# openclimatefix/graph_weather

Hardware: NVIDIA H100
Metric: forward steps/sec (higher is better)
Workload: dtype f32 (fp16x2-split wgmma, fp32 accumulate)

## Files before the change

### graph_weather_b200/csrc/gw_tc3.cu

```cuda
#include <cuda_bf16.h>
#include <cuda_fp16.h>
#include <cuda_runtime.h>
#include <stdint.h>
#include <stdlib.h>

#include <algorithm>
#include <type_traits>

#include "gw_internal.h"
#include "gw_ops.h"
#include "gw_tc_ptx.cuh"

namespace gw {
namespace t3 {

#ifdef GW_ABLATE
#define ABL3(bit) ((ch.ablate & (bit)) != 0)
#else
#define ABL3(bit) false
#endif
#define GW_INLINE __attribute__((always_inline))
enum { ABL_FENCE = 1, ABL_LOADS = 2, ABL_CONVERT = 4, ABL_STORES = 8, ABL_LN = 16, ABL_WEIGHTS = 128 };

enum { F_ADD0 = 1, F_ADD1 = 2, F_RELU = 4, F_LN = 8, F_RES = 16, F_OUT = 32, F_FEEDS = 64, F_SEG = 128, F_NARROW = 256 };
// ... 42 lines not shown
    for (int k = 0; k < 2; ++k) p[k] = base + (size_t)(uint32_t)__ldg(s.idx + i0 + rl[k]) * ldb;
  } else {
#pragma unroll
    for (int k = 0; k < 2; ++k) p[k] = base + (size_t)(uint32_t)(i0 + rl[k]) * ldb;
  }
}
__device__ __forceinline__ void ld256(const char* p, float* o) {
  asm volatile("ld.global.nc.v4.f32 {%0, %1, %2, %3}, [%8];\n\t"
               "ld.global.nc.v4.f32 {%4, %5, %6, %7}, [%8+16];"
               : "=f"(o[0]), "=f"(o[1]), "=f"(o[2]), "=f"(o[3]), "=f"(o[4]), "=f"(o[5]), "=f"(o[6]), "=f"(o[7])
               : "l"(p));
}
__device__ __forceinline__ void st256(char* p, float a, float b, float c, float d, float e, float f, float g, float h) {
  asm volatile("st.global.v4.f32 [%0], {%1, %2, %3, %4};\n\t"
               "st.global.v4.f32 [%0+16], {%5, %6, %7, %8};" ::"l"(p), "f"(a), "f"(b), "f"(c), "f"(d), "f"(e), "f"(f), "f"(g), "f"(h)
               : "memory");
}
__device__ __forceinline__ void load8(const float* rowp, int col, int width, float* o) {
  const float* p = rowp + col;
  if (col + 8 <= width && (reinterpret_cast<uintptr_t>(p) & 31) == 0) {
    ld256(reinterpret_cast<const char*>(p), o);
  } else if (col + 8 <= width && (reinterpret_cast<uintptr_t>(p) & 15) == 0) {
    const float4 a = __ldg(reinterpret_cast<const float4*>(p)), b = __ldg(reinterpret_cast<const float4*>(p + 4));
    o[0] = a.x, o[1] = a.y, o[2] = a.z, o[3] = a.w, o[4] = b.x, o[5] = b.y, o[6] = b.z, o[7] = b.w;
  } else {
#pragma unroll
    for (int t = 0; t < 8; ++t) o[t] = (col + t < width) ? __ldg(p + t) : 0.f;
  }
}
__device__ __forceinline__ const float* src_row(const RowSrc& s, int b, int i0, int r) {
  const int i = src_gathered(s.kind) ? __ldg(s.idx + i0 + r) : i0 + r;
  return reinterpret_cast<const float*>(src_sample_base(s, b)) + (size_t)(uint32_t)i * (size_t)s.ld;
}
__host__ __device__ constexpr int FR(int m, int t) { return 4 * (t >> 1) + 2 * m + (t & 1); }
__host__ __device__ constexpr int PX(int i) { return 8 * ((i >> 1) & 1) + 2 * (i >> 2) + (i & 1); }
__device__ __forceinline__ float4 lds128(uint32_t addr) {
  float4 v;
  asm volatile("ld.shared.v4.f32 {%0, %1, %2, %3}, [%4];" : "=f"(v.x), "=f"(v.y), "=f"(v.z), "=f"(v.w) : "r"(addr));
  return v;
}
__device__ __forceinline__ float col8(const float4& lo, const float4& hi, int i) {
  const int c = 2 * (i >> 2) + (i & 1);
  const float4& b = (c & 4) ? hi : lo;
  return (c & 2) ? ((c & 1) ? b.w : b.z) : ((c & 1) ? b.y : b.x);
}
__device__ __forceinline__ void sts32(uint32_t addr, uint32_t v) { asm volatile("st.shared.b32 [%0], %1;" ::"r"(addr), "r"(v) : "memory"); }
template <bool SPLIT, bool ROWORDER>
__device__ __forceinline__ void store_operand_x4(uint32_t sa, const float (&v)[16], float& amax) {
#pragma unroll
  for (int m = 0; m < 2; ++m)
#pragma unroll
    for (int g = 0; g < 4; ++g) {
      const int i = ROWORDER ? 8 * m + 2 * g : 4 * g + 2 * m;
      const float a0 = v[i], a1 = v[i + 1];
      amax = fmaxf(amax, fmaxf(fabsf(a0), fabsf(a1)));
      const uint32_t addr = (sa ^ (uint32_t)(g << 4)) + 1024u * m;
      if (SPLIT) {
        const __half2 hh = __floats2half2_rn(a0, a1);
        const float2 hf = __half22float2(hh);
        const __half2 ll = __floats2half2_rn(a0 - hf.x, a1 - hf.y);
        sts32(addr, *reinterpret_cast<const uint32_t*>(&hh));
        sts32(addr + A_HALF_BYTES, *reinterpret_cast<const uint32_t*>(&ll));
      } else {
        const __nv_bfloat162 bb = __floats2bfloat162_rn(a0, a1);
        sts32(addr, *reinterpret_cast<const uint32_t*>(&bb));
      }
    }
}

__device__ __forceinline__ float fit_scale(float m) {
  if (!(m > 0.f) || !(m < 3.0e38f)) return 1.f;
  int e = (int)((__float_as_uint(m) >> 23) & 0xffu) - 127;
  e = e < -110 ? -110 : e;
  return __uint_as_float((uint32_t)(127 + 14 - e) << 23);
}
__device__ __forceinline__ float ldbound(const float* p) { return p ? __ldg(p) : 0.f; }
__device__ __forceinline__ float srcbound(const RowSrc& s) {
  if (!s.bound) return 0.f;
  const float m = __ldg(s.bound) * s.bound_mul;
  return s.bound_mul_i ? m * (float)max(__ldg(s.bound_mul_i), 1) : m;
}

template <bool SPLIT, int N>
__device__ __forceinline__ void mma_chunks(float (&d)[128], uint32_t a_rows, uint32_t b_base, uint32_t bar_full_b, uint32_t bar_empty_b,
                                           uint32_t& bi, int kc0, int kc1) {
  for (int kc = kc0; kc < kc1; ++kc) {
    const uint32_t a_hi = a_rows + (uint32_t)(kc % A_SLOTS) * A_SLOT_BYTES, a_lo = a_hi + A_HALF_BYTES;
#pragma unroll
    for (int part = 0; part < (SPLIT ? 2 : 1); ++part) {
      const uint32_t stage = bi % B_STAGES, nb = bi / B_STAGES;
      mbar_wait_or_trap(bar_full_b + 8 * stage, nb & 1);
      const uint32_t b = b_base + stage * B_STAGE_BYTES;
      wgmma_fence();
      if (part == 0) {
#pragma unroll
        for (int ks = 0; ks < 4; ++ks) Wgmma<N, !SPLIT>::mma(d, gmma_desc(a_hi + 32 * ks), gmma_desc(b + 32 * ks), (kc | ks) != 0);
        if (SPLIT) {
#pragma unroll
          for (int ks = 0; ks < 4; ++ks) Wgmma<N, !SPLIT>::mma(d, gmma_desc(a_lo + 32 * ks), gmma_desc(b + 32 * ks), 1);
        }
      } else {
#pragma unroll
        for (int ks = 0; ks < 4; ++ks) Wgmma<N, !SPLIT>::mma(d, gmma_desc(a_hi + 32 * ks), gmma_desc(b + 32 * ks), 1);
      }
      wgmma_commit();
      wgmma_wait<0>();
      mbar_arrive(bar_empty_b + 8 * stage);
      ++bi;
    }
  }
  fence_operand(d);
}

template <bool SPLIT, int MODE>
__global__ void __launch_bounds__(NUM_THREADS, 1) gw_chain_tc3_kernel(const __grid_constant__ TcChain ch) {
  extern __shared__ __align__(1024) uint8_t smem[];
  const uint32_t sbase = smem_u32(smem);
  const int warp = threadIdx.x >> 5, lane = threadIdx.x & 31;
  const int rows = ch.rows_per_sample, batch = ch.batch;
  const int tiles_per_sample = (rows + TILE_M - 1) / TILE_M;
  const int num_tiles = tiles_per_sample * batch;
  constexpr int parts = SPLIT ? 2 : 1;

  const uint32_t bar_full_b = sbase + OFF_BAR;
  const uint32_t bar_empty_b = bar_full_b + 8 * B_STAGES;

  if (threadIdx.x == 0) {
    if (sbase & 1023u) {
      if (ch.status) atomicOr(ch.status, 4);
      __trap();
    }
    for (int i = 0; i < B_STAGES; ++i) mbar_init(bar_full_b + 8 * i, 1), mbar_init(bar_empty_b + 8 * i, NUM_WORKERS);
    fence_barrier_init();
  }
  {
    float* par = reinterpret_cast<float*>(smem + OFF_PAR);
    float* lnp = reinterpret_cast<float*>(smem + OFF_LNP);
    int ln_slot = 0;
    for (int l = 0; l < ch.n_layers; ++l) {
      const TcLayer& L = ch.layer[l];
      for (int c = threadIdx.x; c < 256; c += NUM_THREADS) par[l * 256 + c] = (L.bias && c < L.n_valid) ? __ldg(L.bias + c) : 0.f;
      if (L.ln_g) {
        for (int c = threadIdx.x; c < 256; c += NUM_THREADS) {
          lnp[(ln_slot * 2 + 0) * 256 + c] = (c < L.n_valid) ? __ldg(L.ln_g + c) : 0.f;
          lnp[(ln_slot * 2 + 1) * 256 + c] = (c < L.n_valid) ? __ldg(L.ln_b + c) : 0.f;
        }
        ++ln_slot;
      }
    }
  }
  if (threadIdx.x == 32) {
    float* scl = reinterpret_cast<float*>(smem + OFF_SCL);
    float m = fmaxf(srcbound(ch.a0[0]), srcbound(ch.a0[1]));
    if (ch.a0[0].kind == SRC_GATHER_BCAST_RELU) m += ldbound(ch.a0[0].bound2);
    float sc = fit_scale(m);
    bool bad = !(m < 3.0e38f);
    scl[2 * PAR_LAYERS] = sc;
    for (int l = 0; l < ch.n_layers; ++l) {
      const TcLayer& L = ch.layer[l];
      const float wa = ldbound(L.wamax);
      const float winv = L.wamax ? 1.f / tc_weight_scale(wa, ch.split ? 2 : 1) : L.wscale_inv, gain = L.wamax ? (float)L.K * wa : L.gain;
      scl[2 * l] = winv / sc;
      const float pre = fmaf(m, gain, L.off) + srcbound(L.add[0]) + srcbound(L.add[1]);
      float mo = L.ln_g ? L.ln_bound : pre;
      mo += srcbound(L.residual);
      bad = bad || !(mo < 3.0e38f) || !(pre < 3.0e38f);
      if (blockIdx.x == 0) {
        if (L.out_bound) {
          const bool again = l > 0 && ch.layer[l - 1].out_bound == L.out_bound;
          *L.out_bound = again ? fmaxf(*L.out_bound, mo) : mo;
        }
        if (L.seg_bound) *L.seg_bound = mo * L.seg_maxdeg + ldbound(L.seg_add_bound);
      }
      float so = 1.f;
      if (L.feeds_next) {
        m = mo;
        sc = so = fit_scale(m);
      }
      scl[2 * l + 1] = so;
    }
    if (bad && ch.status) atomicOr(ch.status, 8);
  }
  __syncthreads();
  if (warp >= CONSUMER_WARPS) {
    asm volatile("setmaxnreg.dec.sync.aligned.u32 %0;" ::"n"(AUX_REGS));
    if (warp == WARP_PRODUCER && lane == 0) {
      uint32_t bi = 0;
      Tracer tr;
      tr.init(ch.trace, 0, true);
      for (int tile = blockIdx.x; tile < num_tiles; tile += gridDim.x) {
        for (int l = 0; l < ch.n_layers; ++l) {
          const TcLayer& L = ch.layer[l];
          const uint32_t panel = (uint32_t)L.N * 128u;
// ... 86 lines not shown
    row_ptrs2(ch.a0[0], bs, i0, r2, fcofs, pa);
    if constexpr (GBR) {
#pragma unroll
      for (int m = 0; m < 2; ++m) pb[m] = reinterpret_cast<const char*>(ch.a0[0].base2 + (size_t)(uint32_t)(i0 + r2[m]) * (size_t)ch.a0[0].ld2 + fcofs);
    } else if constexpr (NC1 > 0) {
      row_ptrs2(ch.a0[1], bs, i0, r2, fcofs, pb);
    }
    float buf[DEPTH][16] = {};
    float bufb[GBR ? DEPTH : 1][16] = {};
    auto fetch = [&](auto uu) GW_INLINE {
      constexpr int u = decltype(uu)::value, k = (u - U0) % DEPTH;
      if (ABL3(ABL_LOADS)) return;
      if constexpr (GBR) {
        ld256(pa[0] + 128 * u, buf[k]), ld256(pa[1] + 128 * u, buf[k] + 8);
        ld256(pb[0] + 128 * u, bufb[k]), ld256(pb[1] + 128 * u, bufb[k] + 8);
      } else if constexpr (u < 2 * NC0) {
        ld256(pa[0] + 128 * u, buf[k]), ld256(pa[1] + 128 * u, buf[k] + 8);
      } else {
        ld256(pb[0] + 128 * (u - 2 * NC0), buf[k]), ld256(pb[1] + 128 * (u - 2 * NC0), buf[k] + 8);
      }
    };
    static_for<U0, (U1 < U0 + DEPTH ? U1 : U0 + DEPTH)>([&](auto uu) GW_INLINE { fetch(uu); });
    static_for<U0, U1>([&](auto uu) GW_INLINE {
      constexpr int u = decltype(uu)::value, k = (u - U0) % DEPTH;
      float(&cur)[16] = buf[k];
      if constexpr (GBR) {
#pragma unroll
        for (int i = 0; i < 16; ++i) cur[i] = fmaxf(cur[i] + bufb[k][i], 0.f);
      }
      if (a0scale != 1.f) {
#pragma unroll
        for (int i = 0; i < 16; ++i) cur[i] *= a0scale;
      }
      if (!ABL3(ABL_CONVERT)) store_operand_x4<SPLIT, true>(op_addr(u), cur, amax);
      if constexpr (u + DEPTH < U1) fetch(ic<u + DEPTH>{});
    });
    publish();
  };

  auto bias_in_place = [&](float (&acc)[128], int l, int nu, float wsi) GW_INLINE {
    const uint32_t bias_a = sbase + OFF_PAR + l * 1024 + 4 * fcofs;
    static_for<0, 8>([&](auto uu) GW_INLINE {
      constexpr int u = decltype(uu)::value;
      if (u < nu) {
        const float4 bl = lds128(bias_a + 128 * u), bh = lds128(bias_a + 128 * u + 16);
#pragma unroll
        for (int i = 0; i < 16; ++i) acc[16 * u + i] = fmaf(acc[16 * u + i], wsi, col8(bl, bh, i));
      }
    });
  };
  auto ln_stats = [&](float (&acc)[128], int nu, int nval, float (&rs)[2], float (&sh)[2]) GW_INLINE {
    float s[2] = {0.f, 0.f};
    static_for<0, 8>([&](auto uu) GW_INLINE {
      constexpr int u = decltype(uu)::value;
      if (u < nu) {
#pragma unroll
        for (int i = 0; i < 16; ++i) s[(i >> 1) & 1] += acc[16 * u + i];
      }
    });
#pragma unroll
    for (int m = 0; m < 2; ++m) s[m] += __shfl_xor_sync(0xffffffffu, s[m], 1), s[m] += __shfl_xor_sync(0xffffffffu, s[m], 2);
    const float inv = 1.0f / (float)nval;
    const float mean[2] = {s[0] * inv, s[1] * inv};
    float v2[2] = {0.f, 0.f};
    static_for<0, 8>([&](auto uu) GW_INLINE {
      constexpr int u = decltype(uu)::value;
      if (u < nu) {
#pragma unroll
        for (int i = 0; i < 16; ++i) {
          const int m = (i >> 1) & 1;
          const float d = (32 * u + fcofs + 2 * (i >> 2) + (i & 1) < nval) ? acc[16 * u + i] - mean[m] : 0.f;
          v2[m] = fmaf(d, d, v2[m]);
        }
      }
    });
#pragma unroll
    for (int m = 0; m < 2; ++m) {
      v2[m] += __shfl_xor_sync(0xffffffffu, v2[m], 1), v2[m] += __shfl_xor_sync(0xffffffffu, v2[m], 2);
      const float rstd = 1.0f / sqrtf(v2[m] * inv + 1e-5f);
      rs[m] = rstd, sh[m] = -mean[m] * rstd;
    }
  };

  auto layer_fast = [&](float (&acc)[128], auto FLc, auto NPc, int l, int tile, int ln_slot) GW_INLINE {
    constexpr int F = decltype(FLc)::value, NP = decltype(NPc)::value, NU = 2 * NP;
    constexpr bool has_add0 = (F & F_ADD0) != 0, has_add1 = (F & F_ADD1) != 0, has_res = (F & F_RES) != 0, has_out = (F & F_OUT) != 0;
    constexpr bool relu = (F & F_RELU) != 0, has_ln = (F & F_LN) != 0, feeds = (F & F_FEEDS) != 0, has_seg = (F & F_SEG) != 0;
    constexpr bool has0 = has_add0 || has_res;
    const TcLayer& L = ch.layer[l];
    const int bs = tile % batch, i0 = (tile / batch) * TILE_M;
    const int nvalid = min(TILE_M, rows - i0);
    const float wsi = scl[2 * l], osc = scl[2 * l + 1];
    const uint32_t g_a = sbase + OFF_LNP + 4 * fcofs + (ln_slot * 2) * 1024, b_a = g_a + 1024;
    const RowSrc& src0 = has_add0 ? L.add[0] : L.residual;
    const char* p0[2] = {nullptr, nullptr};
    const char* p1[2] = {nullptr, nullptr};
    float pf0[16] = {}, pf1[16] = {};
    const bool ld_on = !ABL3(ABL_LOADS);
    auto ld2 = [&](const char* const(&p)[2], int off, float(&o)[16]) GW_INLINE { ld256(p[0] + off, o), ld256(p[1] + off, o + 8); };
    {
      const int r2[2] = {min(fr0, nvalid - 1), min(fr0 + 1, nvalid - 1)};
      if constexpr (has0) row_ptrs2(src0, bs, i0, r2, fcofs, p0);
      if constexpr (has_add1) row_ptrs2(L.add[1], bs, i0, r2, fcofs, p1);
    }
    if constexpr (has0) {
      if (ld_on) ld2(p0, 0, pf0);
    }
    if constexpr (has_add1) {
      if (ld_on) ld2(p1, 0, pf1);
    }
    int d0 = 0, d1 = 0, dprev_g = 0;
    if constexpr (has_seg) {
      const int32_t* sd = L.seg_dst + i0;
      d0 = (fr0 < nvalid) ? __ldg(sd + fr0) : -1;
      d1 = (fr0 + 1 < nvalid) ? __ldg(sd + fr0 + 1) : -2;
      dprev_g = (lr == 0 && i0 + frow > 0 && frow < nvalid) ? __ldg(sd + frow - 1) : -8;
    }
    bias_in_place(acc, l, NU, wsi);
    float rs[2] = {1.f, 1.f}, sh[2] = {0.f, 0.f};
    if constexpr (has_ln) {
      if (!ABL3(ABL_LN)) ln_stats(acc, NU, 64 * NP, rs, sh);
    }
    char* po = nullptr;
    const size_t ostr = 4 * (size_t)L.ldo;
    const bool st0 = fr0 < nvalid, st1 = fr0 + 1 < nvalid;
    if constexpr (has_out) po = reinterpret_cast<char*>(L.out + ((size_t)bs * rows + i0 + fr0) * (size_t)L.ldo + fcofs);
    bool bb = false, tail_st = false, head_st = false, one_st = false, one_any = false, deep = false;
    float mbf = 1.f, c1f = 0.f, e2f = 0.f, e4f = 0.f, kf = 0.f, k1f = 0.f;
    char* tail_p = nullptr;
    char* carry_p = nullptr;
    const char* add_p = nullptr;
    if constexpr (has_seg) {
      int dprev = __shfl_up_sync(0xffffffffu, d1, 4);
      if (lr == 0) dprev = dprev_g;
      const bool ba = d0 != dprev;
      bb = d1 != d0;
      mbf = bb ? 0.f : 1.f;
      const uint32_t nba = __shfl_down_sync(0xffffffffu, (uint32_t)ba, 4);
      const bool c1 = lr < 7 && !nba;
      const bool k = c1 && !bb;
      const uint32_t k1 = __shfl_down_sync(0xffffffffu, (uint32_t)k, 4), k2 = __shfl_down_sync(0xffffffffu, (uint32_t)k, 8);
      const uint32_t k3 = __shfl_down_sync(0xffffffffu, (uint32_t)k, 12);
      const bool e2 = c1 && k1;
      const bool e4 = e2 && k2 && k3;
      c1f = c1 ? 1.f : 0.f, e2f = e2 ? 1.f : 0.f, e4f = e4 ? 1.f : 0.f, kf = k ? 1.f : 0.f, k1f = (k && k1) ? 1.f : 0.f;
      deep = L.seg_maxdeg > 7;
      carry_p = reinterpret_cast<char*>(L.seg_carry + ((((size_t)bs * tiles_per_sample + (size_t)(i0 / TILE_M)) * 8 + (size_t)(frow >> 4)) * 256 + fcofs));
      if (ba || bb) {
        tail_st = d1 >= 0;
        tail_p = reinterpret_cast<char*>(L.seg_out + ((size_t)bs * L.seg_rows + (size_t)(uint32_t)max(d1, 0)) * (size_t)L.seg_ld + fcofs);
      } else if (lr == 0) {
        tail_st = d1 >= 0;
        tail_p = carry_p;
      }
      head_st = lr == 0 && !ba && bb && d0 >= 0;
      one_st = ba && bb && d0 >= 0;
      one_any = __any_sync(0xffffffffu, one_st);
      if (L.seg_add && (ba || bb) && d1 >= 0)
        add_p = reinterpret_cast<const char*>(L.seg_add + (size_t)(uint32_t)d1 * (size_t)L.seg_ld + fcofs);
    }
    static_for<0, NU>([&](auto uu) GW_INLINE {
      constexpr int u = decltype(uu)::value;
      float v[16];
#pragma unroll
      for (int i = 0; i < 16; ++i) v[i] = acc[16 * u + i];
      [[maybe_unused]] float sadd[8] = {0.f, 0.f, 0.f, 0.f, 0.f, 0.f, 0.f, 0.f};
      if constexpr (has_seg) {
        if (add_p) ld256(add_p + 128 * u, sadd);
      }
      if constexpr (has_add0) {
        if (ld_on) {
#pragma unroll
          for (int i = 0; i < 16; ++i) v[i] += pf0[PX(i)];
        }
      }
      if constexpr (has_add1) {
        if (ld_on) {
#pragma unroll
          for (int i = 0; i < 16; ++i) v[i] += pf1[PX(i)];
        }
      }
      if constexpr (relu) {
#pragma unroll
        for (int i = 0; i < 16; ++i) v[i] = fmaxf(v[i], 0.f);
      }
      if constexpr (has_ln) {
        const float4 gl = lds128(g_a + 128 * u), gh = lds128(g_a + 128 * u + 16);
        const float4 el = lds128(b_a + 128 * u), eh = lds128(b_a + 128 * u + 16);
#pragma unroll
        for (int i = 0; i < 16; ++i) {
          const int m = (i >> 1) & 1;
          v[i] = fmaf(fmaf(v[i], rs[m], sh[m]), col8(gl, gh, i), col8(el, eh, i));
        }
      }
      if constexpr (has_res) {
        if (ld_on) {
#pragma unroll
          for (int i = 0; i < 16; ++i) v[i] += pf0[PX(i)];
        }
      }
      if constexpr (u + 1 < NU) {
        if constexpr (has0) {
          if (ld_on) ld2(p0, 128 * (u + 1), pf0);
        }
        if constexpr (has_add1) {
          if (ld_on) ld2(p1, 128 * (u + 1), pf1);
        }
      }
      if constexpr (has_out) {
        if (!ABL3(ABL_STORES)) {
          if (st0) st256(po + 128 * u, v[FR(0, 0)], v[FR(0, 1)], v[FR(0, 2)], v[FR(0, 3)], v[FR(0, 4)], v[FR(0, 5)], v[FR(0, 6)], v[FR(0, 7)]);
          if (st1) st256(po + ostr + 128 * u, v[FR(1, 0)], v[FR(1, 1)], v[FR(1, 2)], v[FR(1, 3)], v[FR(1, 4)], v[FR(1, 5)], v[FR(1, 6)], v[FR(1, 7)]);
        }
      }
      if constexpr (has_seg) {
        float T[8], H[8];
#pragma unroll
        for (int t = 0; t < 8; ++t) {
          const float xa = v[FR(0, t)], xb = v[FR(1, t)];
          T[t] = fmaf(mbf, xa, xb);
          H[t] = bb ? xa : T[t];
        }
        const bool sts_on = !ABL3(ABL_STORES);
        if (head_st && sts_on) st256(carry_p + 128 * u, H[0], H[1], H[2], H[3], H[4], H[5], H[6], H[7]);
        if (one_any) {
          if (one_st && sts_on) {
            char* dp = reinterpret_cast<char*>(L.seg_out + ((size_t)bs * L.seg_rows + (size_t)(uint32_t)d0) * (size_t)L.seg_ld + fcofs);
            float a1[8] = {0.f, 0.f, 0.f, 0.f, 0.f, 0.f, 0.f, 0.f};
            if (L.seg_add) ld256(reinterpret_cast<const char*>(L.seg_add + (size_t)(uint32_t)d0 * (size_t)L.seg_ld + fcofs) + 128 * u, a1);
            st256(dp + 128 * u, H[0] + a1[0], H[1] + a1[1], H[2] + a1[2], H[3] + a1[3], H[4] + a1[4], H[5] + a1[5], H[6] + a1[6], H[7] + a1[7]);
          }
        }
#pragma unroll
        for (int t = 0; t < 8; ++t) {
          const float h1 = __shfl_down_sync(0xffffffffu, H[t], 4);
          T[t] = fmaf(c1f, h1, T[t]);
          H[t] = fmaf(kf, h1, H[t]);
        }
#pragma unroll
        for (int t = 0; t < 8; ++t) T[t] = fmaf(e2f, __shfl_down_sync(0xffffffffu, H[t], 8), T[t]);
        if (deep) {
#pragma unroll
          for (int t = 0; t < 8; ++t) {
            const float g2 = fmaf(k1f, __shfl_down_sync(0xffffffffu, H[t], 8), H[t]);
            T[t] = fmaf(e4f, __shfl_down_sync(0xffffffffu, g2, 16), T[t]);
          }
        }
        if (tail_st && sts_on)
          st256(tail_p + 128 * u, T[0] + sadd[0], T[1] + sadd[1], T[2] + sadd[2], T[3] + sadd[3], T[4] + sadd[4], T[5] + sadd[5], T[6] + sadd[6],
                T[7] + sadd[7]);
      }
      if constexpr (feeds) {
        if (osc != 1.f) {
#pragma unroll
          for (int i = 0; i < 16; ++i) v[i] *= osc;
        }
        if (!ABL3(ABL_CONVERT)) store_operand_x4<SPLIT, false>(op_addr(u), v, amax);
      }
      tr.ev(700 + 10 * l + u);
    });
    if constexpr (feeds) publish();
  };

  auto layer_out_narrow = [&](float (&acc)[128], int l, int tile) GW_INLINE {
    const TcLayer& L = ch.layer[l];
    const int bs = tile % batch, i0 = (tile / batch) * TILE_M;
    const int nvalid = min(TILE_M, rows - i0);
    const int nu = L.N >> 5, nval = L.n_valid;
    const bool has_res = L.residual.kind != SRC_NONE;
    const float* rp[2] = {nullptr, nullptr};
    if (has_res) {
      const float* base = reinterpret_cast<const float*>(src_sample_base(L.residual, bs));
#pragma unroll
      for (int m = 0; m < 2; ++m) rp[m] = base + (size_t)(uint32_t)(i0 + min(fr0 + m, nvalid - 1)) * (size_t)L.residual.ld;
    }
    float* op[2];
#pragma unroll
    for (int m = 0; m < 2; ++m) op[m] = L.out + ((size_t)bs * rows + i0 + fr0 + m) * (size_t)L.ldo;
    const bool st[2] = {fr0 < nvalid, fr0 + 1 < nvalid};
    bias_in_place(acc, l, nu, scl[2 * l]);
    static_for<0, 8>([&](auto uu) GW_INLINE {
      constexpr int u = decltype(uu)::value;
      const int c0 = 32 * u + fcofs;
      if (u < nu && 32 * u < nval) {
        float2 r[2][4] = {};
        if (has_res && !ABL3(ABL_LOADS)) {
#pragma unroll
          for (int m = 0; m < 2; ++m)
#pragma unroll
// ... 77 lines not shown
          *reinterpret_cast<float*>(reinterpret_cast<char*>(p) + (reinterpret_cast<const char*>(ch.out_peer[j]) - reinterpret_cast<const char*>(L.out))) = a;
      }
    };
    static_for<0, 8>([&](auto uu) GW_INLINE {
      constexpr int u = decltype(uu)::value;
      if (u < nu) {
        const int col = 32 * u + fcofs;
        const bool ld_ok = !ABL3(ABL_LOADS);
        float v[16];
#pragma unroll
        for (int i = 0; i < 16; ++i) v[i] = acc[16 * u + i];
        float t[16];
        if (has_add0 && ld_ok) {
          load8(q0[0], col, src0.width, t), load8(q0[1], col, src0.width, t + 8);
#pragma unroll
          for (int i = 0; i < 16; ++i) v[i] += t[PX(i)];
        }
        if (has_add1 && ld_ok) {
          load8(q1[0], col, L.add[1].width, t), load8(q1[1], col, L.add[1].width, t + 8);
#pragma unroll
          for (int i = 0; i < 16; ++i) v[i] += t[PX(i)];
        }
        if (relu) {
#pragma unroll
          for (int i = 0; i < 16; ++i) v[i] = fmaxf(v[i], 0.f);
        }
        if (has_pre && !ABL3(ABL_STORES)) store8(L.save_pre, v, col);
        if (has_ln) {
          const float4 gl = lds128(g_a + 128 * u), gh = lds128(g_a + 128 * u + 16);
          const float4 el = lds128(b_a + 128 * u), eh = lds128(b_a + 128 * u + 16);
#pragma unroll
          for (int i = 0; i < 16; ++i) {
            const int m = (i >> 1) & 1;
            v[i] = fmaf(fmaf(v[i], rs[m], sh[m]), col8(gl, gh, i), col8(el, eh, i));
          }
        }
        if (!has_add0 && has_res && ld_ok) {
          load8(q0[0], col, src0.width, t), load8(q0[1], col, src0.width, t + 8);
#pragma unroll
          for (int i = 0; i < 16; ++i) v[i] += t[PX(i)];
        }
        if (has_mask) {
          load8(src_row(L.mask, bs, i0, r2[0]), col, L.mask.width, t), load8(src_row(L.mask, bs, i0, r2[1]), col, L.mask.width, t + 8);
#pragma unroll
          for (int i = 0; i < 16; ++i) v[i] = t[PX(i)] > 0.f ? v[i] : 0.f;
        }
        if (nval < L.N) {
#pragma unroll
          for (int i = 0; i < 16; ++i)
            if (col + 2 * (i >> 2) + (i & 1) >= nval) v[i] = 0.f;
        }
        if (has_out && !ABL3(ABL_STORES)) {
#pragma unroll
          for (int m = 0; m < 2; ++m) {
            if (fr0 + m < nvalid) {
              float* orow = L.out + ((size_t)bs * rows + i0 + fr0 + m) * (size_t)L.ldo + col;
              if (col + 8 <= L.out_cols && (reinterpret_cast<uintptr_t>(orow) & 15) == 0) {
                put4(orow, v[FR(m, 0)], v[FR(m, 1)], v[FR(m, 2)], v[FR(m, 3)]);
                put4(orow + 4, v[FR(m, 4)], v[FR(m, 5)], v[FR(m, 6)], v[FR(m, 7)]);
              } else {
#pragma unroll
                for (int k = 0; k < 8; ++k)
                  if (col + k < L.out_cols) put1(orow + k, v[FR(m, k)]);
              }
            }
          }
        }
        if (feeds) {
          if (osc != 1.f) {
#pragma unroll
            for (int i = 0; i < 16; ++i) v[i] *= osc;
          }
          if (!ABL3(ABL_CONVERT)) store_operand_x4<SPLIT, false>(op_addr(u), v, amax);
        }
      }
    });
    if (feeds) publish();
  };

  auto run_layer = [&](auto Nc, int l, int tile, int ln_slot) GW_INLINE {
    constexpr int N = decltype(Nc)::value;
    const TcLayer& L = ch.layer[l];
    float acc[128];
    auto mma = [&](int kc0, int kc1) GW_INLINE {
      tr.ev(100 + kc0);
      mma_chunks<SPLIT, N>(acc, a_rows, sbase + OFF_B, bar_full_b, bar_empty_b, bi, kc0, kc1);
      wg_sync();
      tr.ev(110 + kc0);
    };
    if (l == 0) {
      const int nk0 = ch.K0 >> 6;
      for (int w = 0; 4 * w < nk0; ++w) {
        tr.ev(480 + w);
        if constexpr (MODE >= 1) {
          if (ch.a0[1].kind != SRC_NONE) {
            if (w == 0) stage0_fast(ic<4>{}, ic<4>{}, ic<0>{}, ic<0>{}, tile);
            else stage0_fast(ic<4>{}, ic<4>{}, ic<0>{}, ic<1>{}, tile);
          } else if (ch.a0[0].kind == SRC_GATHER_BCAST_RELU) {
            stage0_fast(ic<4>{}, ic<0>{}, ic<1>{}, ic<0>{}, tile);
          } else if (ch.K0 == 256) {
            stage0_fast(ic<4>{}, ic<0>{}, ic<0>{}, ic<0>{}, tile);
          } else {
            stage0_fast(ic<2>{}, ic<0>{}, ic<0>{}, ic<0>{}, tile);
          }
        } else {
          stage0(tile, w);
        }
        mma(4 * w, min(nk0, 4 * w + 4));
      }
    } else {
      mma(0, L.K >> 6);
    }
    if constexpr (MODE >= 1) {
      if constexpr (MODE == 2) {
        if (L.kind & F_NARROW) {
          layer_out_narrow(acc, l, tile);
          return;
        }
      }
#define GW_LF(M, NP_) case (M): layer_fast(acc, ic<(M)>{}, ic<(NP_)>{}, l, tile, ln_slot); break
      if constexpr (N == 256) {
        switch (L.kind) {
          GW_LF(F_ADD0 | F_ADD1 | F_RELU | F_FEEDS, 4);
          GW_LF(F_ADD0 | F_RELU | F_FEEDS, 4);
          GW_LF(F_RELU | F_FEEDS, 4);
          GW_LF(F_LN | F_RES | F_OUT, 4);
          GW_LF(F_LN | F_RES | F_OUT | F_SEG, 4);
          GW_LF(F_LN | F_RES | F_SEG, 4);
          GW_LF(F_LN | F_SEG, 4);
          GW_LF(F_LN | F_RES | F_OUT | F_FEEDS, 4);
          GW_LF(F_LN | F_FEEDS, 4);
          GW_LF(F_OUT, 4);
          GW_LF(F_RELU | F_OUT, 4);
          default: break;
        }
      } else {
        switch (L.kind) {
          GW_LF(F_RELU | F_FEEDS, 2);
          GW_LF(F_RELU | F_OUT, 2);
          default: break;
        }
      }
#undef GW_LF
    } else {
      layer_gen(acc, l, tile, ln_slot, l + 1 == ch.n_layers);
    }
  };

  const int n_layers = ch.n_layers;
  for (int tile = blockIdx.x; tile < num_tiles; tile += gridDim.x) {
    int ln_slot = 0;
    for (int l = 0; l < n_layers; ++l) {
      const int N = ch.layer[l].N;
      if constexpr (MODE >= 1) {
        if (N == 256) run_layer(ic<256>{}, l, tile, ln_slot);
        else run_layer(ic<128>{}, l, tile, ln_slot);
      } else {
        if (N == 256) run_layer(ic<256>{}, l, tile, ln_slot);
        else if (N == 192) run_layer(ic<192>{}, l, tile, ln_slot);
        else if (N == 128) run_layer(ic<128>{}, l, tile, ln_slot);
        else run_layer(ic<64>{}, l, tile, ln_slot);
      }
      if (ch.layer[l].ln_g) ++ln_slot;
      tr.ev(900 + l);
    }
  }
  if (SPLIT && ch.status && amax > 60000.f) atomicOr(ch.status, 1);
}

}

static bool aligned32(const void* p) { return (reinterpret_cast<uintptr_t>(p) & 31) == 0; }
static bool simple_kind(int k) { return k == SRC_STREAM || k == SRC_BCAST || k == SRC_GATHER || k == SRC_BGATHER; }
static bool fits32(const RowSrc& s) {
  const bool g = s.kind == SRC_GATHER || s.kind == SRC_BGATHER || s.kind == SRC_GATHER_BCAST_RELU;
  const long long span = g ? (long long)s.src_rows : 128;
  return span * (long long)s.ld * 4 + 4096 < (1ll << 32);
}
static bool src_fast(const RowSrc& s, int need) {
  return simple_kind(s.kind) && s.width >= need && aligned32(s.base + s.col0) && !(s.ld & 7) && fits32(s);
}

static void tc3_mark_lean(TcChain& ch) {
  using namespace t3;
  ch.fast = 0;
  {
    bool ok = true;
    int wsum = 0;
    for (int a = 0; a < 2; ++a) {
      const RowSrc& s = ch.a0[a];
      if (s.kind == SRC_NONE) continue;
      const bool gbr = s.kind == SRC_GATHER_BCAST_RELU;
      ok = ok && (simple_kind(s.kind) || gbr) && aligned32(s.base + s.col0) && !(s.ld & 7);
      if (gbr) ok = ok && aligned32(s.base2) && !(s.ld2 & 7);
      wsum += s.width;
    }
    const bool two = ch.a0[1].kind != SRC_NONE;
    ok = ok && ch.a0[0].kind != SRC_NONE && wsum == ch.K0;
    ok = ok && (two ? (ch.a0[0].width == 256 && ch.a0[1].width == 256) : (ch.K0 == 256 || ch.K0 == 128));
    if (ch.a0[0].kind == SRC_GATHER_BCAST_RELU) ok = ok && !two && ch.K0 == 256;
    if (ok) ch.fast |= (int32_t)0x80000000u;
  }
  static const int kinds4[] = {F_ADD0 | F_ADD1 | F_RELU | F_FEEDS, F_ADD0 | F_RELU | F_FEEDS, F_RELU | F_FEEDS, F_LN | F_RES | F_OUT,
                               F_LN | F_RES | F_OUT | F_SEG, F_LN | F_RES | F_SEG, F_LN | F_SEG, F_LN | F_RES | F_OUT | F_FEEDS, F_LN | F_FEEDS, F_OUT,
                               F_RELU | F_OUT};
  static const int kinds2[] = {F_RELU | F_FEEDS, F_RELU | F_OUT};
  for (int l = 0; l < ch.n_layers; ++l) {
    const TcLayer& L = ch.layer[l];
    if (L.save_pre || L.mask.kind != SRC_NONE) {
      ch.layer[l].kind = -1;
      continue;
    }
    const bool narrow = l + 1 == ch.n_layers && L.n_valid < L.N32 && !(L.n_valid & 1) && (L.N32 == 128 || L.N32 == 256) && L.out && !L.relu &&
                        !L.ln_g && !L.feeds_next && !L.seg_dst && L.add[0].kind == SRC_NONE && L.add[1].kind == SRC_NONE &&
                        !(reinterpret_cast<uintptr_t>(L.out) & 7) && !(L.ldo & 1) && L.out_cols >= L.n_valid &&
                        (L.residual.kind == SRC_NONE ||
                         ((L.residual.kind == SRC_STREAM || L.residual.kind == SRC_BCAST) && L.residual.width >= L.n_valid && !(L.residual.ld & 1) &&
                          !(reinterpret_cast<uintptr_t>(L.residual.base + L.residual.col0) & 7) && fits32(L.residual)));
    if (narrow) {
      ch.layer[l].kind = F_NARROW | F_OUT | (L.residual.kind != SRC_NONE ? F_RES : 0);
      ch.fast |= 1 << l;
      continue;
    }
    bool ok = (L.N == 256 || L.N == 128) && L.n_valid == L.N;
    for (int a = 0; a < 2; ++a)
      if (L.add[a].kind != SRC_NONE) ok = ok && src_fast(L.add[a], L.N);
    if (L.residual.kind != SRC_NONE) ok = ok && src_fast(L.residual, L.N);
    if (L.out) ok = ok && aligned32(L.out) && !(L.ldo & 7) && L.out_cols >= L.N;
    if (L.seg_dst) ok = ok && L.seg_out && L.seg_carry && aligned32(L.seg_out) && aligned32(L.seg_carry) && !(L.seg_ld & 7) && L.ln_g && L.N == 256;
    if (L.seg_add) ok = ok && L.seg_dst && aligned32(L.seg_add);
    const int f = (L.add[0].kind != SRC_NONE ? F_ADD0 : 0) | (L.add[1].kind != SRC_NONE ? F_ADD1 : 0) | (L.relu ? F_RELU : 0) |
                  (L.ln_g ? F_LN : 0) | (L.residual.kind != SRC_NONE ? F_RES : 0) | (L.out ? F_OUT : 0) | (L.feeds_next ? F_FEEDS : 0) |
                  (L.seg_dst ? F_SEG : 0);
    bool listed = false;
    if (L.N == 256) {
      for (int k : kinds4) listed = listed || k == f;
    } else {
      for (int k : kinds2) listed = listed || k == f;
    }
    ch.layer[l].kind = listed ? f : -1;
    if (ok && listed) ch.fast |= 1 << l;
  }
}
bool tc3_chain_is_lean(const TcChain& ch_in) {
  TcChain ch = ch_in;
  tc3_mark_lean(ch);
  if (getenv("GW_TC3_NOFAST")) return false;
  const int32_t all = (int32_t)(0x80000000u | ((1u << ch.n_layers) - 1u));
  return ch.fast == all && ch.out_mode == 0;
}
cudaError_t tc_column_block(const TcChain& ch, int n0, int nb, TcChain* out) {
  const TcLayer& L = ch.layer[0];
  if (ch.n_layers != 1 || n0 < 0 || nb <= 0 || nb > TC_COL_BLOCK || n0 + nb > L.n_valid) return cudaErrorInvalidValue;
  if (L.ln_g && (n0 != 0 || nb != L.n_valid)) return cudaErrorInvalidValue;
  if (L.feeds_next || L.seg_dst || ch.out_mode != 0) return cudaErrorInvalidValue;
  auto shift = [&](RowSrc s) {
    if (s.kind != SRC_NONE) s.col0 += n0, s.width = std::max(0, std::min(s.width - n0, nb));
    return s;
  };
  *out = ch;
  TcLayer& B = out->layer[0];
  B.Wp = nullptr, B.wamax = nullptr;
  B.N = (nb + 15) / 16 * 16, B.N32 = tc_packed_rows(nb), B.n_valid = nb;
  if (L.bias) B.bias = L.bias + n0;
  for (int a = 0; a < 2; ++a) B.add[a] = shift(L.add[a]);
  B.residual = shift(L.residual), B.mask = shift(L.mask);
  if (L.out) B.out = L.out + n0;
  if (L.save_pre) B.save_pre = L.save_pre + n0;
  B.out_cols = std::max(0, std::min(L.out_cols - n0, nb));
  return cudaSuccess;
}
cudaError_t tc_row_op_chain(const GemmOp& op, TcChain* ch) {
  if (op.add[2].kind != SRC_NONE || op.a[0].kind == SRC_NONE || (op.ln_gamma && op.N > TC_COL_BLOCK)) return cudaErrorInvalidValue;
  *ch = TcChain();
  ch->rows_per_sample = op.rows_per_sample, ch->batch = op.batch;
  ch->a0[0] = op.a[0], ch->a0[1] = op.a[1];
  ch->K0 = (op.K + 63) / 64 * 64, ch->n_layers = 1;
  TcLayer& L = ch->layer[0];
  L.K = ch->K0, L.N = op.N, L.n_valid = op.N;
  L.bias = op.bias, L.add[0] = op.add[0], L.add[1] = op.add[1], L.relu = op.relu;
  L.ln_g = op.ln_gamma, L.ln_b = op.ln_beta, L.residual = op.residual;
  L.out = op.out, L.ldo = op.ldo, L.out_cols = op.N, L.save_pre = op.save_pre, L.mask = op.mask;
  return cudaSuccess;
}
cudaError_t launch_operand_bound(RowSrc& s, int rows_per_sample, int batch, float* amax, cudaStream_t st) {
  if (s.kind != SRC_STREAM && s.kind != SRC_BCAST) return cudaErrorInvalidValue;
  const long long n = (long long)(s.kind == SRC_STREAM ? (long long)batch * s.src_rows : (long long)rows_per_sample) * s.ld;
  const cudaError_t e = launch_absmax_flat(s.base, n, amax, st);
  s.bound = amax, s.bound_mul = 1.f, s.bound_mul_i = nullptr;
  return e;
}
float tc_ln_bound(int N, float gamma_amax, float beta_amax) { return sqrtf((float)N) * gamma_amax + beta_amax; }
cudaError_t launch_chain_tc3(const TcChain& ch_in, cudaStream_t stream) {
  TcChain ch = ch_in;
  using namespace t3;
  static int num_sms[64] = {0};
  int dev = 0;
  cudaError_t e = cudaGetDevice(&dev);
  if (e != cudaSuccess) return e;
  if (dev < 0 || dev >= 64) return cudaErrorInvalidDevice;
  if (num_sms[dev] == 0) {
    int n = 0;
    e = cudaDeviceGetAttribute(&n, cudaDevAttrMultiProcessorCount, dev);
    if (e != cudaSuccess) return e;
    const void* fns[6] = {(const void*)gw_chain_tc3_kernel<true, 0>,  (const void*)gw_chain_tc3_kernel<true, 1>,  (const void*)gw_chain_tc3_kernel<true, 2>,
                          (const void*)gw_chain_tc3_kernel<false, 0>, (const void*)gw_chain_tc3_kernel<false, 1>, (const void*)gw_chain_tc3_kernel<false, 2>};
    for (int i = 0; i < 6; ++i) {
      e = cudaFuncSetAttribute(fns[i], cudaFuncAttributeMaxDynamicSharedMemorySize, SMEM_BYTES);
      if (e != cudaSuccess) return e;
    }
    num_sms[dev] = n;
  }
  const long long R = (long long)ch.rows_per_sample * ch.batch;
  if (R <= 0 || ch.n_layers <= 0) return cudaSuccess;
  if (ch.n_layers > PAR_LAYERS || ch.K0 <= 0 || (ch.K0 & 63)) return cudaErrorInvalidValue;
  int n_ln = 0;
  if (ch.a0[1].kind != SRC_NONE && (ch.a0[0].width & 63)) return cudaErrorInvalidValue;
  if (ch.layer[ch.n_layers - 1].feeds_next) return cudaErrorInvalidValue;

  for (int l = 0; l < ch.n_layers; ++l) {
    const TcLayer& L = ch.layer[l];
    if (!L.Wp || (L.K & 63) || (L.N & 15) || L.N > 256 || L.N <= 0 || L.n_valid <= 0 || L.n_valid > L.N) return cudaErrorInvalidValue;
    if (L.feeds_next && (L.N & 63)) return cudaErrorInvalidValue;
    if (L.ln_g && L.add[0].kind != SRC_NONE) return cudaErrorInvalidValue;
    if (L.ln_g && (L.n_valid != L.N || ++n_ln > 2)) return cudaErrorInvalidValue;
    if (L.add[0].kind == SRC_NONE && L.add[1].kind != SRC_NONE) return cudaErrorInvalidValue;
    for (int a = 0; a < 2; ++a)
      if (L.add[a].kind != SRC_NONE && L.add[a].kind != SRC_STREAM && L.add[a].kind != SRC_BCAST && L.add[a].kind != SRC_GATHER &&
          L.add[a].kind != SRC_BGATHER)
        return cudaErrorInvalidValue;
    if (L.residual.kind != SRC_NONE && L.residual.kind != SRC_STREAM && L.residual.kind != SRC_BCAST && L.residual.kind != SRC_GATHER &&
        L.residual.kind != SRC_BGATHER)
      return cudaErrorInvalidValue;
    if (L.add[0].kind != SRC_NONE && L.residual.kind != SRC_NONE) return cudaErrorInvalidValue;
    if (L.mask.kind != SRC_NONE && L.mask.kind != SRC_STREAM && L.mask.kind != SRC_BCAST && L.mask.kind != SRC_GATHER && L.mask.kind != SRC_BGATHER)
      return cudaErrorInvalidValue;
    if (l == 0 && L.K != ch.K0) return cudaErrorInvalidValue;
    if (l > 0 && !L.reuse_a && (!ch.layer[l - 1].feeds_next || ch.layer[l - 1].N != L.K)) return cudaErrorInvalidValue;
    if (L.reuse_a && (l == 0 || L.K != ch.layer[l - 1].K || ch.layer[l - 1].feeds_next || L.K > 64 * A_SLOTS)) return cudaErrorInvalidValue;
  }
  const int tiles = ((ch.rows_per_sample + TILE_M - 1) / TILE_M) * ch.batch;
  const int grid = tiles < num_sms[dev] ? tiles : num_sms[dev];
  tc3_mark_lean(ch);
  if (getenv("GW_TC3_NOFAST")) ch.fast = 0;
  const int32_t all = (int32_t)(0x80000000u | ((1u << ch.n_layers) - 1u));
  int mode = ch.fast == all ? 1 : 0;
  if (ch.out_mode != 0) mode = 0;
  for (int l = 0; l < ch.n_layers; ++l) {
    if (ch.layer[l].N32 < ch.layer[l].N || (ch.layer[l].N32 & 63) || ch.layer[l].N32 > 256) return cudaErrorInvalidValue;
    ch.layer[l].N = ch.layer[l].N32;
  }
  if (mode == 0)
    for (int l = 0; l < ch.n_layers; ++l)
      if (ch.layer[l].seg_dst) return cudaErrorInvalidValue;
  for (int a = 0; a < 2; ++a)
    if (ch.a0[a].kind == SRC_SEGSUM) return cudaErrorInvalidValue;
#define GW_LAUNCH3(SPLIT_, MODE_) gw_chain_tc3_kernel<SPLIT_, MODE_><<<grid, NUM_THREADS, SMEM_BYTES, stream>>>(ch)
  if (mode == 1 && (ch.layer[ch.n_layers - 1].kind & F_NARROW)) mode = 2;
  if (ch.split) {
    if (mode == 2) GW_LAUNCH3(true, 2); else if (mode == 1) GW_LAUNCH3(true, 1); else GW_LAUNCH3(true, 0);
  } else {
    if (mode == 2) GW_LAUNCH3(false, 2); else if (mode == 1) GW_LAUNCH3(false, 1); else GW_LAUNCH3(false, 0);
  }
#undef GW_LAUNCH3
  count_launch();
  return cudaGetLastError();
}

}
```

Measured before the change: 44.97.

## Defer final wgmma wait so epilogue prefetches overlap MMA; deepen operand lookahead

```diff
diff --git a/graph_weather_b200/csrc/gw_tc3.cu b/graph_weather_b200/csrc/gw_tc3.cu
--- a/graph_weather_b200/csrc/gw_tc3.cu
+++ b/graph_weather_b200/csrc/gw_tc3.cu
@@ -148,8 +148,8 @@
 }
 
 template <bool SPLIT, int N>
-__device__ __forceinline__ void mma_chunks(float (&d)[128], uint32_t a_rows, uint32_t b_base, uint32_t bar_full_b, uint32_t bar_empty_b,
-                                           uint32_t& bi, int kc0, int kc1) {
+__device__ __forceinline__ void mma_issue(float (&d)[128], uint32_t a_rows, uint32_t b_base, uint32_t bar_full_b, uint32_t bar_empty_b,
+                                          uint32_t& bi, int kc0, int kc1) {
   for (int kc = kc0; kc < kc1; ++kc) {
     const uint32_t a_hi = a_rows + (uint32_t)(kc % A_SLOTS) * A_SLOT_BYTES, a_lo = a_hi + A_HALF_BYTES;
 #pragma unroll
@@ -170,11 +170,17 @@
         for (int ks = 0; ks < 4; ++ks) Wgmma<N, !SPLIT>::mma(d, gmma_desc(a_hi + 32 * ks), gmma_desc(b + 32 * ks), 1);
       }
       wgmma_commit();
-      wgmma_wait<0>();
-      mbar_arrive(bar_empty_b + 8 * stage);
       ++bi;
-    }
-  }
+      if (part + 1 < (SPLIT ? 2 : 1) || kc + 1 < kc1) {
+        wgmma_wait<0>();
+        mbar_arrive(bar_empty_b + 8 * stage);
+      }
+    }
+  }
+}
+__device__ __forceinline__ void mma_retire(float (&d)[128], uint32_t bar_empty_b, uint32_t bi) {
+  wgmma_wait<0>();
+  mbar_arrive(bar_empty_b + 8 * ((bi + B_STAGES - 1) % B_STAGES));
   fence_operand(d);
 }
 
@@ -427,7 +433,7 @@
     }
   };
 
-  auto layer_fast = [&](float (&acc)[128], auto FLc, auto NPc, int l, int tile, int ln_slot) GW_INLINE {
+  auto layer_fast = [&](float (&acc)[128], auto FLc, auto NPc, int l, int tile, int ln_slot, auto&& retire) GW_INLINE {
     constexpr int F = decltype(FLc)::value, NP = decltype(NPc)::value, NU = 2 * NP;
     constexpr bool has_add0 = (F & F_ADD0) != 0, has_add1 = (F & F_ADD1) != 0, has_res = (F & F_RES) != 0, has_out = (F & F_OUT) != 0;
     constexpr bool relu = (F & F_RELU) != 0, has_ln = (F & F_LN) != 0, feeds = (F & F_FEEDS) != 0, has_seg = (F & F_SEG) != 0;
@@ -440,7 +446,8 @@
     const RowSrc& src0 = has_add0 ? L.add[0] : L.residual;
     const char* p0[2] = {nullptr, nullptr};
     const char* p1[2] = {nullptr, nullptr};
-    float pf0[16] = {}, pf1[16] = {};
+    constexpr int LOOK = has_add1 ? 2 : 1;
+    float pf0[LOOK][16] = {}, pf1[has_add1 ? LOOK : 1][16] = {};
     const bool ld_on = !ABL3(ABL_LOADS);
     auto ld2 = [&](const char* const(&p)[2], int off, float(&o)[16]) GW_INLINE { ld256(p[0] + off, o), ld256(p[1] + off, o + 8); };
     {
@@ -448,12 +455,15 @@
       if constexpr (has0) row_ptrs2(src0, bs, i0, r2, fcofs, p0);
       if constexpr (has_add1) row_ptrs2(L.add[1], bs, i0, r2, fcofs, p1);
     }
-    if constexpr (has0) {
-      if (ld_on) ld2(p0, 0, pf0);
-    }
-    if constexpr (has_add1) {
-      if (ld_on) ld2(p1, 0, pf1);
-    }
+    static_for<0, (LOOK < NU ? LOOK : NU)>([&](auto kk) GW_INLINE {
+      constexpr int k = decltype(kk)::value;
+      if constexpr (has0) {
+        if (ld_on) ld2(p0, 128 * k, pf0[k]);
+      }
+      if constexpr (has_add1) {
+        if (ld_on) ld2(p1, 128 * k, pf1[k]);
+      }
+    });
     int d0 = 0, d1 = 0, dprev_g = 0;
     if constexpr (has_seg) {
       const int32_t* sd = L.seg_dst + i0;
@@ -461,6 +471,7 @@
       d1 = (fr0 + 1 < nvalid) ? __ldg(sd + fr0 + 1) : -2;
       dprev_g = (lr == 0 && i0 + frow > 0 && frow < nvalid) ? __ldg(sd + frow - 1) : -8;
     }
+    retire();
     bias_in_place(acc, l, NU, wsi);
     float rs[2] = {1.f, 1.f}, sh[2] = {0.f, 0.f};
     if constexpr (has_ln) {
@@ -516,13 +527,13 @@
       if constexpr (has_add0) {
         if (ld_on) {
 #pragma unroll
-          for (int i = 0; i < 16; ++i) v[i] += pf0[PX(i)];
+          for (int i = 0; i < 16; ++i) v[i] += pf0[u % LOOK][PX(i)];
         }
       }
       if constexpr (has_add1) {
         if (ld_on) {
 #pragma unroll
-          for (int i = 0; i < 16; ++i) v[i] += pf1[PX(i)];
+          for (int i = 0; i < 16; ++i) v[i] += pf1[u % LOOK][PX(i)];
         }
       }
       if constexpr (relu) {
@@ -541,15 +552,15 @@
       if constexpr (has_res) {
         if (ld_on) {
 #pragma unroll
-          for (int i = 0; i < 16; ++i) v[i] += pf0[PX(i)];
-        }
-      }
-      if constexpr (u + 1 < NU) {
+          for (int i = 0; i < 16; ++i) v[i] += pf0[u % LOOK][PX(i)];
+        }
+      }
+      if constexpr (u + LOOK < NU) {
         if constexpr (has0) {
-          if (ld_on) ld2(p0, 128 * (u + 1), pf0);
+          if (ld_on) ld2(p0, 128 * (u + LOOK), pf0[u % LOOK]);
         }
         if constexpr (has_add1) {
-          if (ld_on) ld2(p1, 128 * (u + 1), pf1);
+          if (ld_on) ld2(p1, 128 * (u + LOOK), pf1[u % LOOK]);
         }
       }
       if constexpr (has_out) {
@@ -793,15 +804,21 @@
     constexpr int N = decltype(Nc)::value;
     const TcLayer& L = ch.layer[l];
     float acc[128];
-    auto mma = [&](int kc0, int kc1) GW_INLINE {
+    int kc_last = 0;
+    auto issue = [&](int kc0, int kc1) GW_INLINE {
       tr.ev(100 + kc0);
-      mma_chunks<SPLIT, N>(acc, a_rows, sbase + OFF_B, bar_full_b, bar_empty_b, bi, kc0, kc1);
+      mma_issue<SPLIT, N>(acc, a_rows, sbase + OFF_B, bar_full_b, bar_empty_b, bi, kc0, kc1);
+      kc_last = kc0;
+    };
+    auto retire = [&]() GW_INLINE {
+      mma_retire(acc, bar_empty_b, bi);
       wg_sync();
-      tr.ev(110 + kc0);
+      tr.ev(110 + kc_last);
     };
     if (l == 0) {
       const int nk0 = ch.K0 >> 6;
       for (int w = 0; 4 * w < nk0; ++w) {
+        if (w > 0) retire();
         tr.ev(480 + w);
         if constexpr (MODE >= 1) {
           if (ch.a0[1].kind != SRC_NONE) {
@@ -817,19 +834,20 @@
         } else {
           stage0(tile, w);
         }
-        mma(4 * w, min(nk0, 4 * w + 4));
+        issue(4 * w, min(nk0, 4 * w + 4));
       }
     } else {
-      mma(0, L.K >> 6);
+      issue(0, L.K >> 6);
     }
     if constexpr (MODE >= 1) {
       if constexpr (MODE == 2) {
         if (L.kind & F_NARROW) {
+          retire();
           layer_out_narrow(acc, l, tile);
           return;
         }
       }
-#define GW_LF(M, NP_) case (M): layer_fast(acc, ic<(M)>{}, ic<(NP_)>{}, l, tile, ln_slot); break
+#define GW_LF(M, NP_) case (M): layer_fast(acc, ic<(M)>{}, ic<(NP_)>{}, l, tile, ln_slot, retire); break
       if constexpr (N == 256) {
         switch (L.kind) {
           GW_LF(F_ADD0 | F_ADD1 | F_RELU | F_FEEDS, 4);
@@ -843,17 +861,18 @@
           GW_LF(F_LN | F_FEEDS, 4);
           GW_LF(F_OUT, 4);
           GW_LF(F_RELU | F_OUT, 4);
-          default: break;
+          default: retire(); break;
         }
       } else {
         switch (L.kind) {
           GW_LF(F_RELU | F_FEEDS, 2);
           GW_LF(F_RELU | F_OUT, 2);
-          default: break;
+          default: retire(); break;
         }
       }
 #undef GW_LF
     } else {
+      retire();
       layer_gen(acc, l, tile, ln_slot, l + 1 == ch.n_layers);
     }
   };
@@ -1002,6 +1021,56 @@
   return e;
 }
 float tc_ln_bound(int N, float gamma_amax, float beta_amax) { return sqrtf((float)N) * gamma_amax + beta_amax; }
+
+struct RowSpan {
+  const char* p = nullptr;
+  long long n = 0, ld = 0, w = 0;
+};
+static RowSpan span_of(const RowSrc& s, long long rows_per_sample, int batch) {
+  RowSpan r;
+  if (s.kind == SRC_NONE || !s.base) return r;
+  const long long n = s.kind == SRC_BCAST ? rows_per_sample : s.kind == SRC_BGATHER ? s.src_rows : (long long)batch * s.src_rows;
+  r.p = reinterpret_cast<const char*>(s.base + s.col0), r.n = n, r.ld = s.ld, r.w = s.width;
+  return r;
+}
+static bool rows_apart(const RowSpan& s, const RowSpan& o, bool same_rows) {
+  if (!s.p || !o.p || s.n <= 0 || o.n <= 0) return true;
+  const char *s_end = s.p + 4 * ((s.n - 1) * s.ld + s.w), *o_end = o.p + 4 * ((o.n - 1) * o.ld + o.w);
+  if (s_end <= o.p || o_end <= s.p) return true;
+  if (s.ld != o.ld || s.ld <= 0) return false;
+  if (s.p == o.p && same_rows) return true;
+  const long long row = 4 * s.ld;
+  long long off = (long long)(s.p - o.p) % row;
+  if (off < 0) off += row;
+  return off >= 4 * o.w && off + 4 * s.w <= row;
+}
+static bool lean_reads_apart(const TcChain& ch) {
+  const long long R = ch.rows_per_sample;
+  RowSpan src[4 + 4 * t3::PAR_LAYERS];
+  bool row_for_row[4 + 4 * t3::PAR_LAYERS];
+  int n = 0;
+  auto push = [&](const RowSpan& r, bool same) { src[n] = r, row_for_row[n++] = same; };
+  auto add = [&](const RowSrc& s) {
+    if (s.kind == SRC_NONE) return;
+    push(span_of(s, R, ch.batch), s.kind == SRC_STREAM && s.src_rows == ch.rows_per_sample);
+    if (s.kind == SRC_GATHER_BCAST_RELU && s.base2) push(RowSpan{reinterpret_cast<const char*>(s.base2), R, s.ld2, s.width}, false);
+  };
+  for (int a = 0; a < 2; ++a) add(ch.a0[a]);
+  for (int l = 0; l < ch.n_layers; ++l) {
+    const TcLayer& L = ch.layer[l];
+    add(L.add[0]), add(L.add[1]), add(L.residual);
+    if (L.seg_add) push(RowSpan{reinterpret_cast<const char*>(L.seg_add), L.seg_rows, L.seg_ld, L.N}, false);
+  }
+  for (int l = 0; l < ch.n_layers; ++l) {
+    const TcLayer& L = ch.layer[l];
+    const RowSpan outs[2] = {L.out ? RowSpan{reinterpret_cast<const char*>(L.out), R * ch.batch, L.ldo, L.out_cols} : RowSpan{},
+                             L.seg_out ? RowSpan{reinterpret_cast<const char*>(L.seg_out), (long long)L.seg_rows * ch.batch, L.seg_ld, L.N} : RowSpan{}};
+    for (int k = 0; k < 2; ++k)
+      for (int i = 0; i < n; ++i)
+        if (!rows_apart(src[i], outs[k], k == 0 && row_for_row[i])) return false;
+  }
+  return true;
+}
 cudaError_t launch_chain_tc3(const TcChain& ch_in, cudaStream_t stream) {
   TcChain ch = ch_in;
   using namespace t3;
@@ -1067,6 +1136,7 @@
   for (int a = 0; a < 2; ++a)
     if (ch.a0[a].kind == SRC_SEGSUM) return cudaErrorInvalidValue;
 #define GW_LAUNCH3(SPLIT_, MODE_) gw_chain_tc3_kernel<SPLIT_, MODE_><<<grid, NUM_THREADS, SMEM_BYTES, stream>>>(ch)
+  if (mode == 1 && !lean_reads_apart(ch)) return cudaErrorInvalidValue;
   if (mode == 1 && (ch.layer[ch.n_layers - 1].kind & F_NARROW)) mode = 2;
   if (ch.split) {
     if (mode == 2) GW_LAUNCH3(true, 2); else if (mode == 1) GW_LAUNCH3(true, 1); else GW_LAUNCH3(true, 0);
```

After: 45.52 (median of 6 runs). 1.2% higher.
